# yangsenwxy/VSR

Hardware: AMD Instinct MI355X
Metric: voxels/sec fwd+bwd, 4× SR on 16×128×128 cine volumes, 1/2/4/8 MI355X (higher is better)
Workload: dtype bf16

## Files before the change

### vsr_amd/csrc/conv_common.h

```cpp
#pragma once
#include "vsrk_common.h"
#include "vsrk_internal.h"
#include <type_traits>

namespace vsrk_conv {


constexpr int NTHR = 512;
constexpr int TW = 32;
constexpr int GTH = 8;
constexpr int ROWB = 80;
constexpr int GTHR = 256;
constexpr int MAXK = 3;

__device__ __forceinline__ int xcd_remap(int bid, int nblk) {
  const int xcd = bid & 7, q = nblk >> 3, rr = nblk & 7;
  const int base = xcd < rr ? xcd * (q + 1) : rr * (q + 1) + (xcd - rr) * q;
  return base + (bid >> 3);
}

struct ConvArgs {
  View x, y, res, msk;
  const char* w;
  const float* bias;
  const float* pro_scale;
  const float* pro_shift;
  int cin, cout, cin_pad, cout_pad;
  int kd, kh, kw, pd, ph, pw;
  int prologue, act, accumulate, has_res, has_mask, xvec, bias_r;
  float out_scale;
  const float* act_param;
  const float* mask_slope;
  int tiles_h, tiles_w, ntn, nblk;
  int ntiles;
};

template <typename T>
__device__ __forceinline__ uint4 mask_tail(uint4 v, int nvalid) {
  constexpr int E = Chunk<T>::E;
  if (nvalid >= E) return v;
  float f[E];
  Chunk<T>::unpack(v, f);
#pragma unroll
  for (int e = 0; e < E; ++e) f[e] = e < nvalid ? f[e] : 0.f;
  return Chunk<T>::pack(f);
}

template <typename T>
__device__ __forceinline__ uint4 load_raw(const View& v, int n, int d, int h, int w, int c, int cin, bool vec) {
  constexpr int E = Chunk<T>::E;
  const T* p = reinterpret_cast<const T*>(v.ptr) + view_off(v, n, d, h, w, c);
  if (vec && c + E <= cin) return *reinterpret_cast<const uint4*>(p);
  float f[E];
#pragma unroll
  for (int e = 0; e < E; ++e) f[e] = (c + e < cin) ? to_f32<T>(p[e]) : 0.f;
  return Chunk<T>::pack(f);
}

template <typename T>
__device__ __forceinline__ uint4 prologue_lds(uint4 v, int c, bool relu, const float* lsc, const float* lsh) {
  constexpr int E = Chunk<T>::E;
  float f[E];
  Chunk<T>::unpack(v, f);
#pragma unroll
  for (int e = 0; e < E; ++e) {
    float t = fmaf(f[e], lsc[c + e], lsh[c + e]);
    f[e] = relu ? fmaxf(t, 0.f) : t;
  }
  return Chunk<T>::pack(f);
}

__device__ __forceinline__ void stage_prologue(float* lsc, float* lsh, int mode, const float* sc, const float* sh,
                                               int cin, int cpad, int tid, int nthr) {
  for (int i = tid; i < cpad; i += nthr) {
    const bool ok = i < cin;
    const bool aff = (mode & VSRK_PRO_AFFINE) != 0;
    lsc[i] = ok ? (aff ? sc[i] : 1.f) : 0.f;
    lsh[i] = ok ? (aff ? sh[i] : 0.f) : 0.f;
  }
}

__device__ __forceinline__ void glds16(const void* gsrc, uint32_t lds_base) {
  unsigned keep;
  asm volatile(
      "s_mov_b32 %0, m0\n\t"
      "s_mov_b32 m0, %2\n\t"
      "s_nop 0\n\t"
      "global_load_lds_dwordx4 %1, off\n\t"
      "s_mov_b32 m0, %0"
      : "=&s"(keep)
      : "v"(gsrc), "s"(lds_base)
      : "memory");
}
#pragma clang diagnostic push
#pragma clang diagnostic ignored "-Winline-asm"
__device__ __forceinline__ void glds16_m0(const void* gsrc, uint32_t lds_base) {
  asm volatile(
      "s_mov_b32 m0, %1\n\t"
      "s_nop 0\n\t"
      "global_load_lds_dwordx4 %0, off"
      :
      : "v"(gsrc), "s"(lds_base)
      : "memory", "m0");
}
#pragma clang diagnostic pop
__device__ __forceinline__ uint32_t lds_addr(const void* p) {
  return (uint32_t)(uintptr_t)(const __attribute__((address_space(3))) char*)(p);
}

__device__ __forceinline__ float act_apply(int act, float t, float slope) {
  if (act == VSRK_ACT_RELU) return fmaxf(t, 0.f);
  if (act == VSRK_ACT_PRELU) return t > 0.f ? t : slope * t;
  return t;
}
__device__ __forceinline__ float mask_apply(float m, float t, float mslope) {
  return m > 0.f ? t : (mslope != 0.f ? mslope * t : 0.f);
}

template <typename T>
__device__ __forceinline__ void mma(f32x16& acc, uint4 a, uint4 b);
template <>
__device__ __forceinline__ void mma<bf16>(f32x16& acc, uint4 a, uint4 b) {
  acc = __builtin_amdgcn_mfma_f32_32x32x16_bf16(__builtin_bit_cast(bf16x8, a),
                                                __builtin_bit_cast(bf16x8, b), acc, 0, 0, 0);
}
template <>
__device__ __forceinline__ void mma<f16>(f32x16& acc, uint4 a, uint4 b) {
  acc = __builtin_amdgcn_mfma_f32_32x32x16_f16(__builtin_bit_cast(f16x8, a), __builtin_bit_cast(f16x8, b), acc, 0,
                                               0, 0);
}
template <>
__device__ __forceinline__ void mma<float>(f32x16& acc, uint4 a, uint4 b) {
  acc = __builtin_amdgcn_mfma_f32_32x32x2f32(__builtin_bit_cast(float, a.x), __builtin_bit_cast(float, b.x), acc, 0, 0, 0);
  acc = __builtin_amdgcn_mfma_f32_32x32x2f32(__builtin_bit_cast(float, a.y), __builtin_bit_cast(float, b.y), acc, 0, 0, 0);
  acc = __builtin_amdgcn_mfma_f32_32x32x2f32(__builtin_bit_cast(float, a.z), __builtin_bit_cast(float, b.z), acc, 0, 0, 0);
  acc = __builtin_amdgcn_mfma_f32_32x32x2f32(__builtin_bit_cast(float, a.w), __builtin_bit_cast(float, b.w), acc, 0, 0, 0);
}

template <typename H> struct V8;
template <> struct V8<bf16> { typedef bf16x8 type; };
template <> struct V8<f16> { typedef f16x8 type; };
__device__ __forceinline__ f32x16 mfma32x16(bf16x8 a, bf16x8 b, f32x16 c) {
  return __builtin_amdgcn_mfma_f32_32x32x16_bf16(a, b, c, 0, 0, 0);
}
__device__ __forceinline__ f32x16 mfma32x16(f16x8 a, f16x8 b, f32x16 c) {
  return __builtin_amdgcn_mfma_f32_32x32x16_f16(a, b, c, 0, 0, 0);
}

template <typename YT, typename Pk>
__device__ __forceinline__ Pk load_pk(const char* base, int64_t off, bool vec, int valid) {
  const YT* p = reinterpret_cast<const YT*>(base) + off;
  if (vec) return *reinterpret_cast<const Pk*>(p);
  Pk v;
  YT* q = reinterpret_cast<YT*>(&v);
  for (int e = 0; e < 4; ++e) q[e] = e < valid ? p[e] : from_f32<YT>(0.f);
  return v;
}
template <typename YT, typename Pk>
__device__ __forceinline__ void unpack_pk(Pk v, float* f) {
  const YT* q = reinterpret_cast<const YT*>(&v);
#pragma unroll
  for (int e = 0; e < 4; ++e) f[e] = to_f32<YT>(q[e]);
}
template <typename YT>
__device__ __forceinline__ void unpack_pk(uint2 v, float* f) { unpack_pk<YT, uint2>(v, f); }
template <typename YT>
__device__ __forceinline__ void unpack_pk(uint4 v, float* f) { unpack_pk<YT, uint4>(v, f); }
template <typename YT, typename Pk>
__device__ __forceinline__ Pk pack_pk(const float* f) {
  Pk v;
  YT* q = reinterpret_cast<YT*>(&v);
#pragma unroll
  for (int e = 0; e < 4; ++e) q[e] = from_f32<YT>(f[e]);
  return v;
}

template <typename YT>
__device__ __forceinline__ void load4(const char* base, int64_t off, bool vec, int valid, float* v) {
  const YT* p = reinterpret_cast<const YT*>(base) + off;
  if (vec) {
    if constexpr (sizeof(YT) == 4) {
      float4 t = *reinterpret_cast<const float4*>(p);
      v[0] = t.x; v[1] = t.y; v[2] = t.z; v[3] = t.w;
    } else {
      uint2 t = *reinterpret_cast<const uint2*>(p);
      const YT* b = reinterpret_cast<const YT*>(&t);
      for (int e = 0; e < 4; ++e) v[e] = to_f32<YT>(b[e]);
    }
  } else {
    for (int e = 0; e < 4; ++e) v[e] = e < valid ? to_f32<YT>(p[e]) : 0.f;
  }
}

struct WgradArgs {
  View x, dy;
  const float* pro_scale;
  const float* pro_shift;
  float* ws;
  int cin, cout;
  int kd, kh, kw, pd, ph, pw;
  int prologue, xvec, dyvec;
  int tiles_h, tiles_w, ntiles, tiles_per_split, nsplit, ncombos, nblk;
  int n_ci_chunks, n_co_tiles, kd_bias, slab, want_bias, cin_pad;
  int sp_by;
  uint16_t sptap[64];
};

typedef short v4i16 __attribute__((ext_vector_type(4)));
typedef __attribute__((address_space(3))) v4i16 lds_v4i16;

__device__ __forceinline__ v4i16 ds_read_tr(const char* p) {
  return __builtin_amdgcn_ds_read_tr16_b64_v4i16((lds_v4i16*)(p));
}

}



static inline bool chunk_ok(const vsrk_tensor5* t, int esize) {
  const int epc = 16 / esize;
  const int r = t->shuffle > 1 ? t->shuffle : 1;
  const bool block_ok = r == 1 || (t->c / (r * r)) % epc == 0;
  const bool stride_ok = t->sw >= epc || (t->w == 1);
  return ((uintptr_t)t->ptr) % 16 == 0 && t->sn % epc == 0 && t->sd % epc == 0 && t->sh % epc == 0 &&
         t->sw % epc == 0 && block_ok && stride_ok;
}

static inline uint16_t subpixel_tapmask(int32_t code, int r, int sub) {
  if (code == 0) return 0x1ff;
  const int k = code & 0xff, sp = (code >> 8) & 0xff, p = (code >> 16) & 0xff;
  const bool tr = (code >> 24) & 1, flip = (code >> 25) & 1;
  if (sp != r) return 0x1ff;
  const int si = sub / r, sj = sub % r;
  auto row = [&](int tap, int ph) { return tr ? sp * (1 - tap) + ph + p : sp * (tap - 1) + ph + p; };
  uint16_t m = 0;
  for (int kh = 0; kh < 3; ++kh)
    for (int kw = 0; kw < 3; ++kw) {
      const int th = flip ? 2 - kh : kh, tw = flip ? 2 - kw : kw;
      const int ky = row(th, si), kx = row(tw, sj);
      if (ky >= 0 && ky < k && kx >= 0 && kx < k) m |= (uint16_t)(1u << (kh * 3 + kw));
    }
  return m;
}

int vsrk_conv_wgrad_pipe(const vsrk_conv::WgradArgs& a, int nco, int nci, int dtype, hipStream_t s);
bool vsrk_wgrad_roll_plan(const vsrk_conv_desc* d, const vsrk_tensor5* x, const vsrk_tensor5* dy, int* nsplit,
                          int* tps, int* ntiles, int* dzc, size_t* ws_bytes);
int vsrk_conv_wgrad_roll(const vsrk_conv_desc* d, const vsrk_tensor5* x, const vsrk_tensor5* dy,
                         const float* pro_scale, const float* pro_shift, int want_bias, float* ws, size_t ws_bytes,
                         int* nsplit_out, hipStream_t s);
void vsrk_conv_set_wgrad_roll_mode(int mode);
extern int vsrk_g_roll_dz;
struct VsrkRowPlan {
  int bands, band_h, nseg, ncot, ncic, nsplit;
  int cot_w, slab;
  size_t ws_bytes;
};
bool vsrk_wgrad_row_plan(const vsrk_conv_desc* d, const vsrk_tensor5* x, const vsrk_tensor5* dy, VsrkRowPlan* p);
int vsrk_conv_wgrad_row(const vsrk_conv_desc* d, const vsrk_tensor5* x, const vsrk_tensor5* dy, int want_bias,
                        float* ws, size_t ws_bytes, VsrkRowPlan* plan, hipStream_t s);
void vsrk_conv_set_wgrad_row_mode(int mode);
int vsrk_conv_wgrad_thin(const vsrk_conv::WgradArgs& a, int nco, int nci, int perm_r, int dtype, hipStream_t s);

static inline bool view_ok(const vsrk_tensor5* t, const char* what) {
  if (!t || !t->ptr) {
    vsrk_set_error("%s: null view", what);
    return false;
  }
  const int r = t->shuffle > 1 ? t->shuffle : 1;
  if (t->c % (r * r) != 0 || (r > 1 && (t->c / (r * r)) % 8 != 0)) {
    vsrk_set_error("%s: sub-pixel view needs channels divisible by 8*shuffle^2 (c=%d, r=%d)", what, t->c, r);
    return false;
  }
  return true;
}
```

### vsr_amd/csrc/conv_fast.hip

```cpp
#include <cstdlib>
#include <string>
#include "conv_fast_impl.h"

namespace {
using namespace vsrk_conv;

int g_fast_mode = -1;

int num_cus_fast() {
  static int n = 0;
  if (n == 0) {
    int dev = 0;
    (void)hipGetDevice(&dev);
    if (hipDeviceGetAttribute(&n, hipDeviceAttributeMultiprocessorCount, dev) != hipSuccess || n <= 0) n = 256;
  }
  return n;
}

}

int vsrk_g_grid_cap = 0;

int vsrk_conv::fast_grid(int64_t ntiles) {
  int64_t g = std::min<int64_t>(ntiles, (int64_t)num_cus_fast());
  if (vsrk_g_grid_cap > 0) g = std::min<int64_t>(g, vsrk_g_grid_cap);
  return (int)std::max<int64_t>(g, 1);
}

extern "C" int vsrk_conv_set_algo(int32_t mode) {
  VSRK_CHECK(mode >= -1 && mode <= 1, "conv_set_algo: mode must be -1, 0 or 1");
  g_fast_mode = mode;
  return VSRK_OK;
}

extern int g_pw_wide_mode;

extern "C" int vsrk_conv_set_path(const char* path, int32_t mode) {
  VSRK_CHECK(path, "conv_set_path: null path");
  const std::string p(path);
  VSRK_CHECK(mode >= -1 && mode <= (p == "wgrad_row" || p == "roll_wr" ? 2 : 1),
             "conv_set_path: mode must be -1, 0 or 1 (wgrad_row, roll_wr: 2)");
  if (p == "fast") g_fast_mode = mode;
  else if (p == "thin") vsrk_g_thin_mode = mode;
  else if (p == "wgrad_pipe") vsrk_g_wgrad_pipe_mode = mode;
  else if (p == "pw") vsrk_g_pw_mode = mode;
  else if (p == "roll") vsrk_conv_set_roll_mode(mode);
  else if (p == "wgrad_roll") vsrk_conv_set_wgrad_roll_mode(mode);
  else if (p == "wgrad_row") vsrk_conv_set_wgrad_row_mode(mode);
  else if (p == "roll_wr") vsrk_conv_set_roll_wr_mode(mode);
  else if (p == "roll_fold") vsrk_conv_set_roll_fold_mode(mode);
  else if (p == "stencil") vsrk_conv_set_stencil_mode(mode);
  else if (p == "pw_wide") g_pw_wide_mode = mode;
  else if (p == "row") vsrk_conv_set_row_mode(mode);
  else VSRK_CHECK(false, "conv_set_path: unknown path '%s' (fast, pw, pw_wide, roll, roll_wr, roll_fold, row, thin, wgrad_pipe, wgrad_roll, wgrad_row, stencil)",
                  path);
  return VSRK_OK;
}

extern "C" int vsrk_conv_set_grid_cap(int32_t max_workgroups) {
  VSRK_CHECK(max_workgroups >= 0, "conv_set_grid_cap: max_workgroups must be >= 0");
  vsrk_g_grid_cap = max_workgroups;
  return VSRK_OK;
}

int vsrk_conv_fwd_fast(const vsrk_conv_desc* d, const vsrk_tensor5* x, const void* w_packed, const float* bias,
                       const float* pro_scale, const float* pro_shift, const vsrk_tensor5* residual,
                       const vsrk_tensor5* mask, const vsrk_tensor5* y, hipStream_t s) {
  if (g_fast_mode < 0) {
    const char* e = getenv("VSRK_CONV_FAST");
    g_fast_mode = (e && e[0] == '0') ? 0 : 1;
  }
  if (g_fast_mode == 0) return 0;
  if (!vsrk_is16(x->dtype)) return 0;
  if (const int rl = vsrk_conv_fwd_roll(d, x, w_packed, bias, pro_scale, pro_shift, residual, mask, y, s)) return rl;
  if (!chunk_ok(x, 2) || x->c % 8 != 0) return 0;
  const int xr = x->shuffle > 1 ? x->shuffle : 1, yr = y->shuffle > 1 ? y->shuffle : 1;
  if (xr > 1 && (x->c / (xr * xr)) % 32 != 0) return 0;
  if (yr > 1 && ((y->c / (yr * yr)) % 32 != 0 || residual || mask)) return 0;
  if (xr > 1 && d->prologue) return 0;
  if (d->kh != d->kw || (d->kh != 1 && d->kh != 3)) return 0;
  const int ye = vsrk_esize(y->dtype);
  if (((uintptr_t)y->ptr) % (4 * ye) != 0 || y->sn % 4 || y->sd % 4 || y->sh % 4 || y->sw % 4) return 0;
  if (y->c % 4 != 0 && !(y->c < 4 && !residual && !mask && !d->accumulate)) return 0;
  for (const vsrk_tensor5* t : {residual, mask}) {
    if (t && (((uintptr_t)t->ptr) % (4 * ye) != 0 || t->sn % 4 || t->sd % 4 || t->sh % 4 || t->sw % 4 ||
              t->shuffle > 1 || t->dtype != y->dtype))
      return 0;
  }
  FastArgs a;
  static int ablate = -1;
  if (ablate < 0) {
    const char* e = getenv("VSRK_FAST_ABLATE");
    ablate = e ? atoi(e) : 0;
  }
  a.ablate = ablate;
  a.x = make_view(x);
  a.y = make_view(y);
  a.res = residual ? make_view(residual) : a.y;
  a.msk = mask ? make_view(mask) : a.y;
  a.w = w_packed;
  a.bias = bias;
  a.pro_scale = pro_scale;
  a.pro_shift = pro_shift;
  a.cin = x->c;
  a.cout = y->c;
  a.cin_pad = round_up(x->c, 32);
  a.cout_pad = round_up(y->c, 128);
  a.kd = d->kd; a.pd = d->pd; a.ph = d->ph; a.pw = d->pw;
  a.prologue = d->prologue;
  a.act = d->act;
  a.accumulate = d->accumulate;
  a.has_res = residual != nullptr;
  a.has_mask = mask != nullptr;
  a.bias_r = d->bias_perm_r;
  a.out_scale = d->out_scale;
  a.act_param = d->act_param;
  a.mask_slope = d->mask_slope;
  a.tiles_w = ceil_div(y->w, TW);
  const int NT = y->c <= 32 ? 32 : (y->c <= 64 || d->kh == 3) ? 64 : 128;
  a.ntn = ceil_div(y->c, NT);
  const bool yf = y->dtype == VSRK_F32;
  const bool h16 = x->dtype == VSRK_F16;
  const bool ys = yr > 1, xs = xr > 1;
  int rc;
  if (d->kh == 1) {
    if (xs || ys) return 0;
    rc = fast_k1(a, NT, yf, h16, s);
  } else if (NT == 32) {
    if (xs || ys) return 0;
    rc = fast_k3_n32(a, yf, h16, s);
  } else if (!xs && !ys) {
    rc = fast_k3_n64(a, yf, h16, s);
  } else if (xs && !ys) {
    rc = fast_k3_n64_xs(a, yf, h16, s);
  } else if (!xs && ys) {
    rc = fast_k3_n64_ys(a, yf, h16, s);
  } else {
    return 0;
  }
  if (rc == kFastNotEligible) return 0;
  return rc == VSRK_OK ? 1 : -rc;
}
```

### vsr_amd/csrc/conv_wgrad_row.hip

```cpp
#include <algorithm>
#include <cstdlib>
#include "conv_common.h"

namespace {
using namespace vsrk_conv;

constexpr int RW_NW = 8;
constexpr int RW_KC = 4;
constexpr int RW_SEG = 32 * RW_KC;
constexpr int RW_XV = RW_SEG + 8;
constexpr int RW_XP = RW_XV / 8;
constexpr int RW_YP = RW_SEG / 8;
constexpr int RW_NP = RW_XP + RW_YP;
constexpr int RW_NQ = (RW_NP + RW_NW - 1) / RW_NW;
constexpr int RW_XSLOT = RW_XP * 1024;
constexpr int RW_YSLOT = RW_YP * 1024;
constexpr int RW_NXS = 4, RW_NYS = 2;
constexpr int RW_YBASE = RW_NXS * RW_XSLOT;
constexpr int RW_LDS = RW_YBASE + RW_NYS * RW_YSLOT;
constexpr int RW_COW = 64;
constexpr int RW_SLAB = 9 * RW_COW * 64 + RW_COW;
constexpr uint32_t RW_OOB = 0x80000000u;

#ifndef RW_ABL
#define RW_ABL 0
#endif

__host__ __device__ constexpr int rw_swz(int j) { return 2 * ((j >> 1) & 1) + 4 * ((j >> 3) & 1); }

typedef __amdgpu_buffer_rsrc_t RwRsrc;
__device__ __forceinline__ RwRsrc rw_rsrc(const void* base) {
  const uint64_t b = (uint64_t)base;
  const uint64_t u = ((uint64_t)(uint32_t)__builtin_amdgcn_readfirstlane((int)(uint32_t)(b >> 32)) << 32) |
                     (uint32_t)__builtin_amdgcn_readfirstlane((int)(uint32_t)b);
  return __builtin_amdgcn_make_buffer_rsrc((void*)u, 0, 0x7FFFFFF0, 0x00020000);
}
typedef uint32_t rw_u32x4 __attribute__((ext_vector_type(4)));
__device__ __forceinline__ void rw_st16(uint32_t addr, uint4 v) {
  *(__attribute__((address_space(3))) rw_u32x4*)(size_t)addr = __builtin_bit_cast(rw_u32x4, v);
}

typedef float f32x4_t __attribute__((ext_vector_type(4)));
template <typename H> struct V8R;
template <> struct V8R<bf16> { typedef bf16x8 type; };
template <> struct V8R<f16> { typedef f16x8 type; };
__device__ __forceinline__ f32x4_t rw_mfma(bf16x8 a, bf16x8 b, f32x4_t c) {
  return __builtin_amdgcn_mfma_f32_16x16x32_bf16(a, b, c, 0, 0, 0);
}
__device__ __forceinline__ f32x4_t rw_mfma(f16x8 a, f16x8 b, f32x4_t c) {
  return __builtin_amdgcn_mfma_f32_16x16x32_f16(a, b, c, 0, 0, 0);
}
__device__ __forceinline__ uint4 rw_frag(uint32_t p0, uint32_t p1) {
  const v4i16 a = __builtin_amdgcn_ds_read_tr16_b64_v4i16((lds_v4i16*)(size_t)p0);
  const v4i16 b = __builtin_amdgcn_ds_read_tr16_b64_v4i16((lds_v4i16*)(size_t)p1);
  return __builtin_bit_cast(uint4, __builtin_shufflevector(a, b, 0, 1, 2, 3, 4, 5, 6, 7));
}

constexpr int RW_MAXB = 16;

struct RowArgs {
  const char* x;
  const char* dy;
  int xoff[RW_MAXB], yoff[RW_MAXB];
  uint16_t tapm[RW_MAXB];
  int tapm_x;
  float* ws;
  int64_t xsn, xsd, xsh, xsw, ysn, ysd, ysh, ysw;
  int xd, H, W;
  int bands, band_h, nseg, ncot, ncic, nsplit;
  int want_bias;
  int prio;
};

template <typename H, bool SPM>
__global__ __launch_bounds__(RW_NW * 64, 1) void wgrad_row_kernel(RowArgs a) {
  using V8 = typename V8R<H>::type;
  extern __shared__ __attribute__((aligned(16))) char lds[];
  const int lane = threadIdx.x & 63;
  const int wave = __builtin_amdgcn_readfirstlane(threadIdx.x >> 6);
  const int coh = wave & 1, cib = wave >> 1;

  const int ncombo = a.ncot * a.ncic;
  const int L = xcd_remap(blockIdx.x, a.nsplit * ncombo);
  const int split = L / ncombo;
  const int combo = L - split * ncombo;
  const int cot = combo % a.ncot, cic = combo / a.ncot;
  const int seg = split % a.nseg;
  const int t0 = split / a.nseg;
  const int band = t0 % a.bands, img = t0 / a.bands;
  const int nb = img / a.xd, dd = img - nb * a.xd;
  const int h0 = band * a.band_h;
  const int nst = min(a.H, h0 + a.band_h) - h0;
  const int w0 = seg * RW_SEG;
  const unsigned tapm = SPM ? (unsigned)a.tapm[a.tapm_x ? cic : cot] : 0x1ffu;
  const char* xim = a.x + 2 * (nb * a.xsn + dd * a.xsd + a.xoff[cic]);
  const char* yim = a.dy + 2 * (nb * a.ysn + dd * a.ysd + a.yoff[cot]);

  static_assert(RW_XP == 2 * RW_NW + 1 && RW_YP == 2 * RW_NW, "piece roles");
  uint32_t goff[RW_NQ], loff[RW_NQ];
#pragma unroll
  for (int q = 0; q < RW_NQ; ++q) {
    const bool isx = q != 2 && q != 3;
    const int j = q == 4 ? 2 * RW_NW : wave + RW_NW * (q & 1);
    if (isx) {
      const int v = 8 * j + (lane >> 3);
      const int col = w0 - 1 + v;
      const bool ok = v < RW_SEG + 2 && col >= 0 && col < a.W;
      goff[q] = ok ? (uint32_t)(2 * (col * (int)a.xsw + 8 * (lane & 7))) : RW_OOB;
      loff[q] = (uint32_t)(j * 1024 + (lane >> 3) * 128 + 16 * ((lane & 7) ^ rw_swz(v)));
    } else {
      const int v = 8 * j + (lane >> 3);
      const int col = w0 + v;
      goff[q] = col < a.W ? (uint32_t)(2 * (col * (int)a.ysw + 8 * (lane & 7))) : RW_OOB;
      loff[q] = (uint32_t)(j * 1024 + (lane >> 3) * 128 + 16 * ((lane & 7) ^ rw_swz(v)));
    }
  }
  const uint32_t lbase = lds_addr(lds);
  auto load_set = [&](int t, uint4 (&r)[RW_NQ]) __attribute__((always_inline)) {
    const int xr = h0 - 1 + t;
    const bool xok = xr >= 0 && xr < a.H;
    const int yr = t - 2;
    const bool yok = yr >= 0 && yr < nst;
    const RwRsrc rx = rw_rsrc(xim + 2 * (int64_t)(xok ? xr : 0) * a.xsh);
    const RwRsrc ry = rw_rsrc(yim + 2 * (int64_t)(h0 + (yok ? yr : 0)) * a.ysh);
#pragma unroll
    for (int q = 0; q < RW_NQ; ++q) {
      const bool isx = q != 2 && q != 3;
      if (q == 4 && wave != 0) break;
      r[q] = __builtin_bit_cast(uint4, __builtin_amdgcn_raw_buffer_load_b128(
                                           isx ? rx : ry, (int)((isx ? xok : yok) ? goff[q] : RW_OOB), 0, 0));
    }
  };
  auto store_set = [&](int t, const uint4 (&r)[RW_NQ]) __attribute__((always_inline)) {
    const uint32_t xs = lbase + (uint32_t)(t % RW_NXS) * RW_XSLOT;
    const int yr = t - 2;
    const uint32_t ys = lbase + RW_YBASE + (uint32_t)((yr < 0 ? 0 : yr) % RW_NYS) * RW_YSLOT;
#pragma unroll
    for (int q = 0; q < RW_NQ; ++q) {
      const bool isx = q != 2 && q != 3;
      if (q == 4 && wave != 0) break;
      if (isx) rw_st16(xs + loff[q], r[q]);
      else if (yr >= 0) rw_st16(ys + loff[q], r[q]);
    }
  };

  const int g = lane >> 4, qq = (lane >> 2) & 3, pp = lane & 3;
  uint32_t xo[3][2];
#pragma unroll
  for (int kw = 0; kw < 3; ++kw)
#pragma unroll
    for (int h = 0; h < 2; ++h) {
      const int v = kw + 8 * g + qq + 4 * h;
      xo[kw][h] = (uint32_t)(v * 128 + 16 * ((2 * cib + (pp >> 1)) ^ rw_swz(v)) + 8 * (pp & 1));
    }
  uint32_t yo[2][2];
#pragma unroll
  for (int b = 0; b < 2; ++b)
#pragma unroll
    for (int h = 0; h < 2; ++h) {
      const int v = 8 * g + qq + 4 * h;
      yo[b][h] = (uint32_t)(v * 128 + 16 * ((2 * (2 * coh + b) + (pp >> 1)) ^ rw_swz(v)) + 8 * (pp & 1));
    }

  f32x4_t acc[3][3][2];
#pragma unroll
  for (int i = 0; i < 18; ++i) acc[i / 6][(i / 2) % 3][i % 2] = f32x4_t{0.f, 0.f, 0.f, 0.f};
  f32x4_t bacc[2] = {f32x4_t{0.f, 0.f, 0.f, 0.f}, f32x4_t{0.f, 0.f, 0.f, 0.f}};
  uint4 ones;
  {
    const H one = from_f32<H>(1.f);
    const uint16_t u = __builtin_bit_cast(uint16_t, one);
    const uint32_t w2 = (uint32_t)u | ((uint32_t)u << 16);
    ones = make_uint4(w2, w2, w2, w2);
  }

  const int last = nst + 1;
  uint4 stg[RW_NQ], stg2[RW_NQ];
  load_set(0, stg);
  if (1 <= last) load_set(1, stg2);
  store_set(0, stg);
  if (1 <= last) store_set(1, stg2);
  if (2 <= last) {
    load_set(2, stg);
    store_set(2, stg);
  }
  __syncthreads();
  if (3 <= last) load_set(3, stg);
  __builtin_amdgcn_sched_barrier(0);

  for (int s = 0; s < nst; ++s) {
    uint32_t xa[3][3][2], ya[2][2];
#pragma unroll
    for (int kh = 0; kh < 3; ++kh) {
      const uint32_t xrow = lbase + (uint32_t)((s + kh) % RW_NXS) * RW_XSLOT;
#pragma unroll
      for (int kw = 0; kw < 3; ++kw)
#pragma unroll
        for (int h = 0; h < 2; ++h) {
          xa[kh][kw][h] = xrow + xo[kw][h];
          asm volatile("" : "+v"(xa[kh][kw][h]));
        }
    }
    {
      const uint32_t yr = lbase + RW_YBASE + (uint32_t)(s % RW_NYS) * RW_YSLOT;
#pragma unroll
      for (int b = 0; b < 2; ++b)
#pragma unroll
        for (int h = 0; h < 2; ++h) {
          ya[b][h] = yr + yo[b][h];
          asm volatile("" : "+v"(ya[b][h]));
        }
    }
    uint4 xf[2][3], yf[2][2];
    auto load_group = [&](int G) __attribute__((always_inline)) {
      const int kc = G / 3, kh = G % 3;
      if (kh == 0) {
#pragma unroll
        for (int b = 0; b < 2; ++b) yf[kc & 1][b] = rw_frag(ya[b][0] + kc * 4096, ya[b][1] + kc * 4096);
      }
#pragma unroll
      for (int kw = 0; kw < 3; ++kw) xf[G & 1][kw] = rw_frag(xa[kh][kw][0] + kc * 4096, xa[kh][kw][1] + kc * 4096);
    };
    load_group(0);
#pragma unroll
    for (int G = 0; G < 3 * RW_KC; ++G) {
      if (G + 1 < 3 * RW_KC) load_group(G + 1);
      __builtin_amdgcn_sched_barrier(0);
      if (a.prio) __builtin_amdgcn_s_setprio(1);
      const int kc = G / 3, kh = G % 3;
#pragma unroll
      for (int kw = 0; kw < 3; ++kw) {
        if (SPM && !((tapm >> (kh * 3 + kw)) & 1)) continue;
#pragma unroll
        for (int b = 0; b < 2; ++b)
          if (RW_ABL & 2) acc[kh][kw][b][0] += __builtin_bit_cast(float, yf[kc & 1][b].x ^ xf[G & 1][kw].y);
          else acc[kh][kw][b] = rw_mfma(__builtin_bit_cast(V8, yf[kc & 1][b]), __builtin_bit_cast(V8, xf[G & 1][kw]),
                                   acc[kh][kw][b]);
      }
      if (kh == 1 && kc == cib) {
#pragma unroll
        for (int b = 0; b < 2; ++b)
          bacc[b] = rw_mfma(__builtin_bit_cast(V8, yf[kc & 1][b]), __builtin_bit_cast(V8, ones), bacc[b]);
      }
      if (a.prio) __builtin_amdgcn_s_setprio(0);
      __builtin_amdgcn_sched_barrier(0);
    }
    if (!(RW_ABL & 1)) {
      if (s + 3 <= last) store_set(s + 3, stg);
      asm volatile("s_waitcnt lgkmcnt(0)\n\ts_barrier" ::: "memory");
      if (s + 4 <= last) load_set(s + 4, stg);
    }
    __builtin_amdgcn_sched_barrier(0);
  }

  float* out = a.ws + ((int64_t)split * ncombo + combo) * RW_SLAB;
  const int l15 = lane & 15, lg = lane >> 4;
#pragma unroll
  for (int t9 = 0; t9 < 9; ++t9)
#pragma unroll
    for (int b = 0; b < 2; ++b)
#pragma unroll
      for (int i = 0; i < 4; ++i) {
        const int co = 32 * coh + 16 * b + 4 * lg + i, ci = 16 * cib + l15;
        out[(t9 * RW_COW + co) * 64 + ci] = ((tapm >> t9) & 1) ? acc[t9 / 3][t9 % 3][b][i] : 0.f;
      }
  if (a.want_bias && cic == 0) {
    float* part = reinterpret_cast<float*>(lds);
    __syncthreads();
    if (l15 == 0) {
#pragma unroll
      for (int b = 0; b < 2; ++b)
#pragma unroll
        for (int i = 0; i < 4; ++i) part[cib * 64 + 32 * coh + 16 * b + 4 * lg + i] = bacc[b][i];
    }
    __syncthreads();
    if (threadIdx.x < RW_COW) {
      const int c = threadIdx.x;
      out[9 * RW_COW * 64 + c] = ((part[c] + part[64 + c]) + part[128 + c]) + part[192 + c];
    }
  }
}

int g_wrow_mode = -1;

int wrow_num_cus() {
  static int n = 0;
  if (n == 0) {
    int dev = 0;
    (void)hipGetDevice(&dev);
    if (hipDeviceGetAttribute(&n, hipDeviceAttributeMultiprocessorCount, dev) != hipSuccess || n <= 0) n = 256;
  }
  return n;
}

}

void vsrk_conv_set_wgrad_row_mode(int mode) { g_wrow_mode = mode; }

bool vsrk_wgrad_row_plan(const vsrk_conv_desc* d, const vsrk_tensor5* x, const vsrk_tensor5* dy, VsrkRowPlan* p) {
  if (g_wrow_mode < 0) {
    const char* e = getenv("VSRK_WGRAD_ROW");
    g_wrow_mode = (e && e[0] == '0') ? 0 : 1;
  }
  if (g_wrow_mode == 0) return false;
  if (!vsrk_is16(x->dtype) || dy->dtype != x->dtype) return false;
  if (d->kd != 1 || d->kh != 3 || d->kw != 3 || d->pd != 0 || d->ph != 1 || d->pw != 1) return false;
  if (d->prologue != VSRK_PRO_NONE) return false;
  if (x->c % 64 || dy->c % 64 || (x->shuffle > 1 && dy->shuffle > 1)) return false;
  if (d->subpixel && (x->shuffle > 1 || dy->shuffle > 1) && g_wrow_mode != 2) return false;
  if (x->c / 64 > RW_MAXB || dy->c / 64 > RW_MAXB) return false;
  for (const vsrk_tensor5* t : {x, dy}) {
    if (t->shuffle <= 1) continue;
    const int r = t->shuffle, cph = t->c / (r * r);
    if (cph * r * r != t->c || cph % 64) return false;
  }
  if (x->n != dy->n || x->d != dy->d || x->h != dy->h || x->w != dy->w) return false;
  if (!chunk_ok(x, 2) || !chunk_ok(dy, 2)) return false;
  for (const vsrk_tensor5* t : {x, dy}) {
    const int64_t r = t->shuffle > 1 ? t->shuffle : 1;
    if (t->sn < 0 || t->sd < 0 || t->sh < 0 || t->sw < 0 ||
        (int64_t)(RW_XV + 2) * r * t->sw + (r - 1) * t->sh + t->c >= (1ll << 29))
      return false;
  }
  const int64_t images = (int64_t)x->n * x->d;
  if (images <= 0 || x->h <= 0 || x->w <= 0) return false;
  const int nseg = ceil_div(x->w, RW_SEG);
  const int ncot = dy->c / RW_COW, ncic = x->c / 64;
  const int64_t per_band = images * nseg * ncot * ncic;
  int64_t want = std::max<int64_t>(1, wrow_num_cus());
  if (vsrk_g_grid_cap > 0) want = std::min<int64_t>(want, vsrk_g_grid_cap);
  int bands = (int)std::max<int64_t>(1, std::min<int64_t>((want + per_band / 2) / per_band, ceil_div(x->h, 8)));
  {
    static int ov = -1;
    if (ov < 0) {
      const char* e = getenv("VSRK_WGRAD_ROW_BANDS");
      ov = e ? std::max(0, atoi(e)) : 0;
    }
    if (ov > 0) bands = std::min(ov, x->h);
  }
  if (vsrk_g_grid_cap > 0) bands = std::max(1, std::min(bands, x->h));
  p->band_h = ceil_div(x->h, bands);
  p->bands = ceil_div(x->h, p->band_h);
  p->nseg = nseg;
  p->ncot = ncot;
  p->ncic = ncic;
  const int64_t ns = images * p->bands * nseg;
  if (ns * ncot * ncic >= (1ll << 30)) return false;
  p->nsplit = (int)ns;
  p->cot_w = RW_COW;
  p->slab = RW_SLAB;
  p->ws_bytes = (size_t)ns * ncot * ncic * RW_SLAB * sizeof(float);
  return true;
}

int vsrk_conv_wgrad_row(const vsrk_conv_desc* d, const vsrk_tensor5* x, const vsrk_tensor5* dy, int want_bias,
                        float* ws, size_t ws_bytes, VsrkRowPlan* plan, hipStream_t s) {
  VsrkRowPlan p;
  if (!vsrk_wgrad_row_plan(d, x, dy, &p)) return 0;
  if (ws_bytes < p.ws_bytes) return 0;
  RowArgs a;
  a.x = (const char*)x->ptr;
  a.dy = (const char*)dy->ptr;
  a.ws = ws;
  auto blocks = [](const vsrk_tensor5* t, int64_t& sh, int64_t& sw, int* off) {
    const int r = t->shuffle > 1 ? t->shuffle : 1;
    sh = (int64_t)r * t->sh;
    sw = (int64_t)r * t->sw;
    const int cph = t->c / (r * r);
    for (int b = 0; b < t->c / 64; ++b) {
      const int c = 64 * b, sub = c / cph, cc = c - sub * cph;
      off[b] = (int)((sub / r) * t->sh + (sub % r) * t->sw + cc);
    }
  };
  a.xsn = x->sn; a.xsd = x->sd;
  a.ysn = dy->sn; a.ysd = dy->sd;
  blocks(x, a.xsh, a.xsw, a.xoff);
  blocks(dy, a.ysh, a.ysw, a.yoff);
  const vsrk_tensor5* spt = x->shuffle > 1 ? x : (dy->shuffle > 1 ? dy : nullptr);
  const bool spm = d->subpixel && spt;
  a.tapm_x = spt == x;
  if (spm) {
    const int r = spt->shuffle, cph = spt->c / (r * r);
    const int32_t code = d->subpixel & ~(1 << 25);
    for (int b = 0; b < spt->c / 64; ++b) a.tapm[b] = (uint16_t)subpixel_tapmask(code, r, 64 * b / cph);
  }
  a.xd = x->d;
  a.H = x->h;
  a.W = x->w;
  a.bands = p.bands;
  a.band_h = p.band_h;
  a.nseg = p.nseg;
  a.ncot = p.ncot;
  a.ncic = p.ncic;
  a.nsplit = p.nsplit;
  a.want_bias = want_bias;
  {
    static int prio = -1;
    if (prio < 0) {
      const char* e = getenv("VSRK_WGRAD_ROW_PRIO");
      prio = (e && e[0] == '1') ? 1 : 0;
    }
    a.prio = prio;
  }
  const int grid = p.nsplit * p.ncot * p.ncic;
  vsrk_dispatch16(x->dtype, [&](auto tag) {
    using H = decltype(tag);
    auto kern = spm ? wgrad_row_kernel<H, true> : wgrad_row_kernel<H, false>;
    (void)hipFuncSetAttribute((const void*)kern, hipFuncAttributeMaxDynamicSharedMemorySize, RW_LDS);
    kern<<<grid, RW_NW * 64, RW_LDS, s>>>(a);
    return 0;
  });
  *plan = p;
  return 1;
}
```

Baseline: 62.84 million.

## Split wgrad row kernel waves by tap group and issue next-stage loads early

Reassigns waves in the row-band weight-gradient kernel. Each wave now covers all 64 output channels for one input-channel block, and the waves are split into two tap groups (taps 0-4 and 5-8, with bias on the second group), instead of two output-channel halves that each cover all nine taps. Each x fragment load is therefore reused across four output blocks, cutting LDS reads per MFMA. It also prefetches three stages in the prologue and moves the next-slab store and global load to the middle of the inner MFMA loop, to overlap memory with compute. Risks include higher register pressure and more y-fragment loads per wave.

```diff
diff --git a/vsr_amd/csrc/conv_common.h b/vsr_amd/csrc/conv_common.h
--- a/vsr_amd/csrc/conv_common.h
+++ b/vsr_amd/csrc/conv_common.h
@@ -260,6 +260,7 @@
 int vsrk_conv_wgrad_row(const vsrk_conv_desc* d, const vsrk_tensor5* x, const vsrk_tensor5* dy, int want_bias,
                         float* ws, size_t ws_bytes, VsrkRowPlan* plan, hipStream_t s);
 void vsrk_conv_set_wgrad_row_mode(int mode);
+void vsrk_conv_set_wgrad_row_split_mode(int mode);
 int vsrk_conv_wgrad_thin(const vsrk_conv::WgradArgs& a, int nco, int nci, int perm_r, int dtype, hipStream_t s);
 
 static inline bool view_ok(const vsrk_tensor5* t, const char* what) {
diff --git a/vsr_amd/csrc/conv_fast.hip b/vsr_amd/csrc/conv_fast.hip
--- a/vsr_amd/csrc/conv_fast.hip
+++ b/vsr_amd/csrc/conv_fast.hip
@@ -38,8 +38,8 @@
 extern "C" int vsrk_conv_set_path(const char* path, int32_t mode) {
   VSRK_CHECK(path, "conv_set_path: null path");
   const std::string p(path);
-  VSRK_CHECK(mode >= -1 && mode <= (p == "wgrad_row" || p == "roll_wr" ? 2 : 1),
-             "conv_set_path: mode must be -1, 0 or 1 (wgrad_row, roll_wr: 2)");
+  VSRK_CHECK(mode >= -1 && mode <= (p == "wgrad_row_split" ? 3 : (p == "wgrad_row" || p == "roll_wr" ? 2 : 1)),
+             "conv_set_path: mode must be -1, 0 or 1 (wgrad_row, roll_wr: 2; wgrad_row_split: 3)");
   if (p == "fast") g_fast_mode = mode;
   else if (p == "thin") vsrk_g_thin_mode = mode;
   else if (p == "wgrad_pipe") vsrk_g_wgrad_pipe_mode = mode;
@@ -47,12 +47,13 @@
   else if (p == "roll") vsrk_conv_set_roll_mode(mode);
   else if (p == "wgrad_roll") vsrk_conv_set_wgrad_roll_mode(mode);
   else if (p == "wgrad_row") vsrk_conv_set_wgrad_row_mode(mode);
+  else if (p == "wgrad_row_split") vsrk_conv_set_wgrad_row_split_mode(mode);
   else if (p == "roll_wr") vsrk_conv_set_roll_wr_mode(mode);
   else if (p == "roll_fold") vsrk_conv_set_roll_fold_mode(mode);
   else if (p == "stencil") vsrk_conv_set_stencil_mode(mode);
   else if (p == "pw_wide") g_pw_wide_mode = mode;
   else if (p == "row") vsrk_conv_set_row_mode(mode);
-  else VSRK_CHECK(false, "conv_set_path: unknown path '%s' (fast, pw, pw_wide, roll, roll_wr, roll_fold, row, thin, wgrad_pipe, wgrad_roll, wgrad_row, stencil)",
+  else VSRK_CHECK(false, "conv_set_path: unknown path '%s' (fast, pw, pw_wide, roll, roll_wr, roll_fold, row, thin, wgrad_pipe, wgrad_roll, wgrad_row, wgrad_row_split, stencil)",
                   path);
   return VSRK_OK;
 }
diff --git a/vsr_amd/csrc/conv_wgrad_row.hip b/vsr_amd/csrc/conv_wgrad_row.hip
--- a/vsr_amd/csrc/conv_wgrad_row.hip
+++ b/vsr_amd/csrc/conv_wgrad_row.hip
@@ -1,5 +1,6 @@
 #include <algorithm>
 #include <cstdlib>
+#include <type_traits>
 #include "conv_common.h"
 
 namespace {
@@ -22,6 +23,9 @@
 constexpr int RW_SLAB = 9 * RW_COW * 64 + RW_COW;
 constexpr uint32_t RW_OOB = 0x80000000u;
 
+#ifndef RW_EARLY_AT
+#define RW_EARLY_AT (NG / 2)
+#endif
 #ifndef RW_ABL
 #define RW_ABL 0
 #endif
@@ -70,15 +74,18 @@
   int bands, band_h, nseg, ncot, ncic, nsplit;
   int want_bias;
   int prio;
+  int pro3;
+  int early;
 };
 
-template <typename H, bool SPM>
+template <typename H, bool SPM, bool SPLIT>
 __global__ __launch_bounds__(RW_NW * 64, 1) void wgrad_row_kernel(RowArgs a) {
   using V8 = typename V8R<H>::type;
   extern __shared__ __attribute__((aligned(16))) char lds[];
   const int lane = threadIdx.x & 63;
   const int wave = __builtin_amdgcn_readfirstlane(threadIdx.x >> 6);
-  const int coh = wave & 1, cib = wave >> 1;
+  const int cib = SPLIT ? wave & 3 : wave >> 1;
+  const int tg = wave >> 2, coh = wave & 1;
 
   const int ncombo = a.ncot * a.ncic;
   const int L = xcd_remap(blockIdx.x, a.nsplit * ncombo);
@@ -153,19 +160,22 @@
       const int v = kw + 8 * g + qq + 4 * h;
       xo[kw][h] = (uint32_t)(v * 128 + 16 * ((2 * cib + (pp >> 1)) ^ rw_swz(v)) + 8 * (pp & 1));
     }
-  uint32_t yo[2][2];
-#pragma unroll
-  for (int b = 0; b < 2; ++b)
+  constexpr int NB = SPLIT ? 4 : 2;
+  const int co0 = SPLIT ? 0 : 32 * coh;
+  uint32_t yo[NB][2];
+#pragma unroll
+  for (int b = 0; b < NB; ++b)
 #pragma unroll
     for (int h = 0; h < 2; ++h) {
       const int v = 8 * g + qq + 4 * h;
-      yo[b][h] = (uint32_t)(v * 128 + 16 * ((2 * (2 * coh + b) + (pp >> 1)) ^ rw_swz(v)) + 8 * (pp & 1));
-    }
-
-  f32x4_t acc[3][3][2];
-#pragma unroll
-  for (int i = 0; i < 18; ++i) acc[i / 6][(i / 2) % 3][i % 2] = f32x4_t{0.f, 0.f, 0.f, 0.f};
-  f32x4_t bacc[2] = {f32x4_t{0.f, 0.f, 0.f, 0.f}, f32x4_t{0.f, 0.f, 0.f, 0.f}};
+      yo[b][h] = (uint32_t)(v * 128 + 16 * ((2 * ((co0 >> 4) + b) + (pp >> 1)) ^ rw_swz(v)) + 8 * (pp & 1));
+    }
+
+  constexpr int NT = SPLIT ? 5 : 9;
+  constexpr int BT = SPLIT ? 4 : 9;
+  f32x4_t acc[SPLIT ? 5 : 10][NB];
+#pragma unroll
+  for (int i = 0; i < (SPLIT ? 5 : 10) * NB; ++i) acc[i / NB][i % NB] = f32x4_t{0.f, 0.f, 0.f, 0.f};
   uint4 ones;
   {
     const H one = from_f32<H>(1.f);
@@ -177,10 +187,16 @@
   const int last = nst + 1;
   uint4 stg[RW_NQ], stg2[RW_NQ];
   load_set(0, stg);
-  if (1 <= last) load_set(1, stg2);
-  store_set(0, stg);
-  if (1 <= last) store_set(1, stg2);
-  if (2 <= last) {
+  load_set(1, stg2);
+  if (a.pro3) {
+    uint4 stg3[RW_NQ];
+    load_set(2, stg3);
+    store_set(0, stg);
+    store_set(1, stg2);
+    store_set(2, stg3);
+  } else {
+    store_set(0, stg);
+    store_set(1, stg2);
     load_set(2, stg);
     store_set(2, stg);
   }
@@ -188,90 +204,129 @@
   if (3 <= last) load_set(3, stg);
   __builtin_amdgcn_sched_barrier(0);
 
-  for (int s = 0; s < nst; ++s) {
-    uint32_t xa[3][3][2], ya[2][2];
-#pragma unroll
-    for (int kh = 0; kh < 3; ++kh) {
-      const uint32_t xrow = lbase + (uint32_t)((s + kh) % RW_NXS) * RW_XSLOT;
-#pragma unroll
-      for (int kw = 0; kw < 3; ++kw)
-#pragma unroll
-        for (int h = 0; h < 2; ++h) {
-          xa[kh][kw][h] = xrow + xo[kw][h];
-          asm volatile("" : "+v"(xa[kh][kw][h]));
-        }
-    }
+  auto stage = [&](auto role, int s) __attribute__((always_inline)) {
+    constexpr int ROLE = decltype(role)::value;
+    constexpr int T0 = ROLE == 2 ? 5 : 0;
+    constexpr int NTR = ROLE == 0 ? 9 : (ROLE == 1 ? 5 : 4);
+    constexpr int NS = ROLE == 0 ? 3 : 2;
+    constexpr int S1 = ROLE == 2 ? 2 : 3;
+    constexpr int NG = NS * RW_KC;
+    uint32_t xa[NTR][2], ya[NB][2];
+    uint32_t xrow[3];
+#pragma unroll
+    for (int kh = 0; kh < 3; ++kh) xrow[kh] = lbase + (uint32_t)((s + kh) % RW_NXS) * RW_XSLOT;
+#pragma unroll
+    for (int lt = 0; lt < NTR; ++lt)
+#pragma unroll
+      for (int h = 0; h < 2; ++h) {
+        xa[lt][h] = xrow[(T0 + lt) / 3] + xo[(T0 + lt) % 3][h];
+        asm volatile("" : "+v"(xa[lt][h]));
+      }
     {
       const uint32_t yr = lbase + RW_YBASE + (uint32_t)(s % RW_NYS) * RW_YSLOT;
 #pragma unroll
-      for (int b = 0; b < 2; ++b)
+      for (int b = 0; b < NB; ++b)
 #pragma unroll
         for (int h = 0; h < 2; ++h) {
           ya[b][h] = yr + yo[b][h];
           asm volatile("" : "+v"(ya[b][h]));
         }
     }
-    uint4 xf[2][3], yf[2][2];
+    uint4 xf[2][3], yf[2][NB];
+    auto sub_t0 = [](int sub) { return sub == 0 ? 0 : (sub == 1 ? S1 : 6); };
+    auto sub_nt = [&](int sub) { return (sub + 1 < NS ? sub_t0(sub + 1) : NTR) - sub_t0(sub); };
     auto load_group = [&](int G) __attribute__((always_inline)) {
-      const int kc = G / 3, kh = G % 3;
-      if (kh == 0) {
-#pragma unroll
-        for (int b = 0; b < 2; ++b) yf[kc & 1][b] = rw_frag(ya[b][0] + kc * 4096, ya[b][1] + kc * 4096);
-      }
-#pragma unroll
-      for (int kw = 0; kw < 3; ++kw) xf[G & 1][kw] = rw_frag(xa[kh][kw][0] + kc * 4096, xa[kh][kw][1] + kc * 4096);
+      const int kc = G / NS, sub = G % NS;
+      if (sub == 0) {
+#pragma unroll
+        for (int b = 0; b < NB; ++b) yf[kc & 1][b] = rw_frag(ya[b][0] + kc * 4096, ya[b][1] + kc * 4096);
+      }
+#pragma unroll
+      for (int j = 0; j < 3; ++j)
+        if (j < sub_nt(sub)) {
+          const int lt = sub_t0(sub) + j;
+          xf[G & 1][j] = rw_frag(xa[lt][0] + kc * 4096, xa[lt][1] + kc * 4096);
+        }
     };
     load_group(0);
 #pragma unroll
-    for (int G = 0; G < 3 * RW_KC; ++G) {
-      if (G + 1 < 3 * RW_KC) load_group(G + 1);
+    for (int G = 0; G < NG; ++G) {
+      if (G + 1 < NG) load_group(G + 1);
+      if (G == RW_EARLY_AT && a.early && !(RW_ABL & 1)) {
+        if (s + 3 <= last) store_set(s + 3, stg);
+        if (s + 4 <= last) load_set(s + 4, stg);
+      }
       __builtin_amdgcn_sched_barrier(0);
       if (a.prio) __builtin_amdgcn_s_setprio(1);
-      const int kc = G / 3, kh = G % 3;
-#pragma unroll
-      for (int kw = 0; kw < 3; ++kw) {
-        if (SPM && !((tapm >> (kh * 3 + kw)) & 1)) continue;
-#pragma unroll
-        for (int b = 0; b < 2; ++b)
-          if (RW_ABL & 2) acc[kh][kw][b][0] += __builtin_bit_cast(float, yf[kc & 1][b].x ^ xf[G & 1][kw].y);
-          else acc[kh][kw][b] = rw_mfma(__builtin_bit_cast(V8, yf[kc & 1][b]), __builtin_bit_cast(V8, xf[G & 1][kw]),
-                                   acc[kh][kw][b]);
-      }
-      if (kh == 1 && kc == cib) {
-#pragma unroll
-        for (int b = 0; b < 2; ++b)
-          bacc[b] = rw_mfma(__builtin_bit_cast(V8, yf[kc & 1][b]), __builtin_bit_cast(V8, ones), bacc[b]);
+      const int kc = G / NS, sub = G % NS;
+#pragma unroll
+      for (int j = 0; j < 3; ++j) {
+        if (j >= sub_nt(sub)) continue;
+        const int lt = sub_t0(sub) + j;
+        if (SPM && !((tapm >> (T0 + lt)) & 1)) continue;
+#pragma unroll
+        for (int b = 0; b < NB; ++b)
+          if (RW_ABL & 2) acc[lt][b][0] += __builtin_bit_cast(float, yf[kc & 1][b].x ^ xf[G & 1][j].y);
+          else acc[lt][b] = rw_mfma(__builtin_bit_cast(V8, yf[kc & 1][b]), __builtin_bit_cast(V8, xf[G & 1][j]),
+                                    acc[lt][b]);
+      }
+      if (ROLE != 1 && sub == 1 && kc == cib) {
+#pragma unroll
+        for (int b = 0; b < NB; ++b)
+          acc[BT][b] = rw_mfma(__builtin_bit_cast(V8, yf[kc & 1][b]), __builtin_bit_cast(V8, ones), acc[BT][b]);
       }
       if (a.prio) __builtin_amdgcn_s_setprio(0);
       __builtin_amdgcn_sched_barrier(0);
     }
-    if (!(RW_ABL & 1)) {
-      if (s + 3 <= last) store_set(s + 3, stg);
-      asm volatile("s_waitcnt lgkmcnt(0)\n\ts_barrier" ::: "memory");
-      if (s + 4 <= last) load_set(s + 4, stg);
-    }
-    __builtin_amdgcn_sched_barrier(0);
+  };
+
+  auto stages = [&](auto role) __attribute__((always_inline)) {
+    for (int s = 0; s < nst; ++s) {
+      stage(role, s);
+      if (!(RW_ABL & 1)) {
+        if (!a.early && s + 3 <= last) store_set(s + 3, stg);
+        asm volatile("s_waitcnt lgkmcnt(0)\n\ts_barrier" ::: "memory");
+        if (!a.early && s + 4 <= last) load_set(s + 4, stg);
+      }
+      __builtin_amdgcn_sched_barrier(0);
+    }
+  };
+  if constexpr (SPLIT) {
+    if (tg == 0) stages(std::integral_constant<int, 1>{});
+    else stages(std::integral_constant<int, 2>{});
+  } else {
+    stages(std::integral_constant<int, 0>{});
   }
 
   float* out = a.ws + ((int64_t)split * ncombo + combo) * RW_SLAB;
   const int l15 = lane & 15, lg = lane >> 4;
-#pragma unroll
-  for (int t9 = 0; t9 < 9; ++t9)
-#pragma unroll
-    for (int b = 0; b < 2; ++b)
-#pragma unroll
-      for (int i = 0; i < 4; ++i) {
-        const int co = 32 * coh + 16 * b + 4 * lg + i, ci = 16 * cib + l15;
-        out[(t9 * RW_COW + co) * 64 + ci] = ((tapm >> t9) & 1) ? acc[t9 / 3][t9 % 3][b][i] : 0.f;
-      }
+  auto write_taps = [&](int t0, int nt) __attribute__((always_inline)) {
+#pragma unroll
+    for (int lt = 0; lt < NT; ++lt) {
+      if (lt >= nt) continue;
+#pragma unroll
+      for (int b = 0; b < NB; ++b)
+#pragma unroll
+        for (int i = 0; i < 4; ++i) {
+          const int co = co0 + 16 * b + 4 * lg + i, ci = 16 * cib + l15;
+          out[((t0 + lt) * RW_COW + co) * 64 + ci] = ((tapm >> (t0 + lt)) & 1) ? acc[lt][b][i] : 0.f;
+        }
+    }
+  };
+  if constexpr (SPLIT) {
+    if (tg == 0) write_taps(0, 5);
+    else write_taps(5, 4);
+  } else {
+    write_taps(0, 9);
+  }
   if (a.want_bias && cic == 0) {
     float* part = reinterpret_cast<float*>(lds);
     __syncthreads();
-    if (l15 == 0) {
-#pragma unroll
-      for (int b = 0; b < 2; ++b)
-#pragma unroll
-        for (int i = 0; i < 4; ++i) part[cib * 64 + 32 * coh + 16 * b + 4 * lg + i] = bacc[b][i];
+    if (l15 == 0 && (!SPLIT || tg == 1)) {
+#pragma unroll
+      for (int b = 0; b < NB; ++b)
+#pragma unroll
+        for (int i = 0; i < 4; ++i) part[cib * 64 + co0 + 16 * b + 4 * lg + i] = acc[BT][b][i];
     }
     __syncthreads();
     if (threadIdx.x < RW_COW) {
@@ -282,6 +337,7 @@
 }
 
 int g_wrow_mode = -1;
+int g_wrow_split = -1;
 
 int wrow_num_cus() {
   static int n = 0;
@@ -296,6 +352,7 @@
 }
 
 void vsrk_conv_set_wgrad_row_mode(int mode) { g_wrow_mode = mode; }
+void vsrk_conv_set_wgrad_row_split_mode(int mode) { g_wrow_split = mode; }
 
 bool vsrk_wgrad_row_plan(const vsrk_conv_desc* d, const vsrk_tensor5* x, const vsrk_tensor5* dy, VsrkRowPlan* p) {
   if (g_wrow_mode < 0) {
@@ -402,10 +459,22 @@
     }
     a.prio = prio;
   }
+  int split = g_wrow_split;
+  if (split < 0) {
+    static int env = -1;
+    if (env < 0) {
+      const char* e = getenv("VSRK_WGRAD_ROW_SPLIT");
+      env = (e && e[0] >= '0' && e[0] <= '3') ? e[0] - '0' : 1;
+    }
+    split = env;
+  }
+  a.pro3 = split != 0;
+  a.early = split == 1 || split == 3;
   const int grid = p.nsplit * p.ncot * p.ncic;
   vsrk_dispatch16(x->dtype, [&](auto tag) {
     using H = decltype(tag);
-    auto kern = spm ? wgrad_row_kernel<H, true> : wgrad_row_kernel<H, false>;
+    auto kern = (split == 1 || split == 2) ? (spm ? wgrad_row_kernel<H, true, true> : wgrad_row_kernel<H, false, true>)
+                      : (spm ? wgrad_row_kernel<H, true, false> : wgrad_row_kernel<H, false, false>);
     (void)hipFuncSetAttribute((const void*)kern, hipFuncAttributeMaxDynamicSharedMemorySize, RW_LDS);
     kern<<<grid, RW_NW * 64, RW_LDS, s>>>(a);
     return 0;
```

Measured after the change: 63.07 million (median of 3 runs). About the same (+0.4%).
